# drprojects/DeepViewAgg

Hardware: AMD Instinct MI355X
Metric: points/sec fused fwd+bwd (1M pts, 32 views) (higher is better)
Workload: dtype bf16

## Files before the change

### deepviewagg_amd/_lib.py

```python
import ctypes
import os

_HERE = os.path.dirname(os.path.abspath(__file__))
LIB_PATH = os.environ.get("DVA_LIB_PATH") or os.path.join(_HERE, "csrc", "libdva_hip.so")

DVA_F32, DVA_BF16, DVA_F16 = 0, 1, 2
DVA_GRID_F32, DVA_GRID_F64, DVA_GRID_I32, DVA_GRID_I64 = 0, 1, 2, 3
DVA_SUM, DVA_MEAN, DVA_MAX, DVA_MIN = 0, 1, 2, 3
REDUCE_CODE = {"sum": DVA_SUM, "add": DVA_SUM, "mean": DVA_MEAN, "max": DVA_MAX, "min": DVA_MIN}
CAMERA_CODE = {
    "s3dis_equirectangular": 0,
    "scannet": 1,
    "kitti360_perspective": 2,
    "kitti360_fisheye": 3,
}

_ERRORS = {
    -1: "DVA_ERR_INVALID (bad argument)",
    -2: "DVA_ERR_UNSUPPORTED",
    -3: "DVA_ERR_LAUNCH (HIP runtime error)",
    -4: "DVA_ERR_OVERFLOW (composite key does not fit int64)",
}
DVA_ERR_UNSUPPORTED = -2

# ... 173 lines not shown
    "dva_copy_ceiling": (ctypes.c_int, [_vp, _vp, _i64, _vp]),
    "dva_zero_unseen_rows": (ctypes.c_int, [_vp, _vp, _i64, _i64, _vp]),
    "dva_chain_bn_consts": (ctypes.c_int, [_vp, ctypes.c_double, _vp, _vp, _vp, _vp, _vp, ctypes.c_float, ctypes.c_float,
                                           _i32, _vp, _i32, _i32, _vp, _vp, _vp]),
    "dva_concat_cast_fwd": (ctypes.c_int, [_vp, _vp, _vp, _i64, _i32, _i32, _i32, _vp]),
    "dva_concat_cast_bwd": (ctypes.c_int, [_vp, _vp, _vp, _i64, _i32, _i32, _i32, _vp]),
    "dva_mapping_row_index": (ctypes.c_int, [_vp, _vp, _vp, _i32, ctypes.c_double, _i64, _i64, _i32, _i32, _i32, _vp, _vp]),
    "dva_view_gather_rows_grad_rec16_to": (ctypes.c_int, [_vp, _vp, _vp, _vp, _vp, _i32, _i64, _i64, _i32, _i32, _i32, _vp]),
    "dva_chain_tile_chunks": (ctypes.c_int, [_vp, _i64, _i64, _i32, _vp, _vp]),
    "dva_chain_tile_offsets": (ctypes.c_int, [_vp, _i32, _vp, _vp, _vp]),
    "dva_bn_bwd_consts": (ctypes.c_int, [_vp, _vp, ctypes.c_double, _i32, _vp, _vp, _vp, _i32, _vp]),
    "dva_chain3_prep": (ctypes.c_int, [_vp, _vp, _vp, _i32, _vp, _vp, _i32, _vp, _vp]),
    "dva_chain3_stats2": (ctypes.c_int, [_vp] * 11 + [_i64, _vp]),
    "dva_chain3_stats": (ctypes.c_int, [_i32] + [_vp] * 9 + [_i64, _i64, _vp]),
    "dva_chain3_scores": (ctypes.c_int, [_vp] * 7 + [_i32, _vp, _i64, _vp]),
    "dva_chain3_score_stats": (ctypes.c_int, [_vp] * 10 + [_i32, _i64, _vp]),
    "dva_chain3_bwd_layer": (ctypes.c_int, [_i32] + [_vp] * 19 + [_i64, _i64, _vp]),
    "dva_chain_stats1": (ctypes.c_int, [_vp, _vp, _i32, _vp, _vp]),
    "dva_chain_dw1": (ctypes.c_int, [_vp, _vp, _vp, _i32, _vp, _vp, _vp, _vp]),
    "dva_chain_set_prep": (ctypes.c_int, [_vp, _i32, _vp, _vp, _i32, _vp, _vp]),
    "dva_chain_set_fwd": (ctypes.c_int, [_i32, _vp, _vp, _vp, _vp, _vp, _vp, _vp, _vp, _i64, _vp]),
    "dva_chain_set_bwd": (ctypes.c_int, [_i32, _vp, _vp, _vp, _vp, _vp, _vp, _vp, _vp, _vp, _vp, _vp, _i32, _vp, _vp,
                                         _i64, _vp]),
    "dva_chain3_set_prep": (ctypes.c_int, [_vp, _i32, _vp, _vp, _i32, _vp, _vp]),
    "dva_chain3_set_fwd": (ctypes.c_int, [_i32, _vp, _vp, _vp, _vp, _vp, _vp, _vp, _vp, _i64, _vp]),
    "dva_chain3_set_bwd": (ctypes.c_int, [_i32, _vp, _vp, _vp, _vp, _vp, _vp, _vp, _vp, _vp, _vp, _vp, _i32, _vp, _vp,
                                         _i64, _vp]),
    "dva_voxel_parent_workspace_bytes": (ctypes.c_int64, [_i64]),
    "dva_voxel_parent_index": (ctypes.c_int, [_vp, _i64, _vp, _i64, _i32, _i32, _vp, _vp, _i64, _vp]),
    "dva_voxel_kernel_map": (ctypes.c_int, [_vp, _i64, _vp, _i64, _vp, _i32, _vp, _vp, _i64, _vp]),
    "dva_sparse_conv_workspace_bytes": (ctypes.c_int64, [_i32, _i32, _i32, _i32]),
    "dva_sparse_conv_apply": (ctypes.c_int, [_vp, _vp, _vp, _vp, _vp, _i64, _i64, _i32, _i32, _i32, _i32, _i32, _vp,
                                             _i64, _vp]),
    "dva_sparse_conv_wgrad": (ctypes.c_int, [_vp, _vp, _vp, _vp, _i64, _i64, _i32, _i32, _i32, _i32, _vp]),
    "dva_knn_workspace_bytes": (ctypes.c_int64, [_i64]),
    "dva_knn": (ctypes.c_int, [_vp, _i64, _vp, _f32, _i32, _i32, _vp, _vp, _vp, _vp, _i64, _vp]),
    "dva_view_occlusion": (ctypes.c_int, [_vp, _vp, _i64, _i64, _i32, _vp, _i32, _vp, _i32, _vp, _vp, _vp]),
    "dva_knn_query_workspace_bytes": (ctypes.c_int64, [_i64, _i64]),
    "dva_knn_query": (ctypes.c_int, [_vp, _i64, _vp, _i64, _vp, _f32, _i32, _i32, _vp, _vp, _vp, _vp, _i64, _vp]),
    "dva_pointwise_pca": (ctypes.c_int, [_vp, _i64, _vp, _i64, _i32, _vp, _vp, _vp]),
    "dva_grid_workspace_bytes": (ctypes.c_int64, [_i64, _i64]),
    "dva_grid_quantize": (ctypes.c_int, [_vp, _i32, _i64, _f64, _vp, _vp, _vp, _vp, _i64, _vp]),
    "dva_grid_cluster": (ctypes.c_int, [_vp, _vp, _vp, _i64, _vp, _i32, _vp, _vp, _vp, _vp, _vp, _vp, _vp, _i64, _vp]),
    "dva_grid_mean": (ctypes.c_int, [_vp, _i32, _i64, _i32, _vp, _vp, _i64, _vp, _vp, _i64, _vp]),
    "dva_grid_majority": (ctypes.c_int, [_vp, _i64, _vp, _i64, _i64, _i64, _i32, _vp, _vp, _i64, _vp]),
    "dva_radius_query_workspace_bytes": (ctypes.c_int64, [_i64, _i64]),
# ... 178 lines not shown
```

### deepviewagg_amd/csrc/chain_set.hip

```cpp
#include "chain_split.h"

namespace dva {
namespace chain {

enum { SO_WSA = 0, SO_WSB = 4, SO_WCB = 8, SO_WCBT = 12, SO_WSBT = 16, SO_WSAT = 20, N_SOPS = 24 };

__global__ __launch_bounds__(64) void set_prep_kernel(const float* __restrict__ Wsa, int ldsa,
                                                      const float* __restrict__ Wsb, const float* __restrict__ Wc,
                                                      int ldc, uint4* __restrict__ ops) {
  const int op = blockIdx.x, lane = threadIdx.x, j = lane & 31, h = lane >> 5;
  const int mat = op / 4, lo = (op >> 1) & 1, m = op & 1;
  float w[8];
#pragma unroll
  for (int s = 0; s < 8; ++s) {
    const int c = chan(8 * m + s, h);
    float v;
    switch (mat) {
      case 0: v = Wsa[j * ldsa + c]; break;
      case 1: v = Wsb[j * D + c]; break;
      case 2: v = Wc[j * ldc + D + c]; break;
      case 3: v = Wc[c * ldc + D + j]; break;
      case 4: v = Wsb[c * D + j]; break;
      default: v = Wsa[c * ldsa + j]; break;
    }
    const float hi = bf2f(f2bf(v));
    w[s] = lo ? v - hi : hi;
  }
  ops[op * 64 + lane] = __builtin_bit_cast(uint4, pack8(w));
}

template <int DIR, int STAGE>
__global__ __launch_bounds__(256, DIR == 0 ? 4 : 3) void set_kernel(
    const float* __restrict__ pooled, const int64_t* __restrict__ ptr, const float* __restrict__ w33,
    const uint4* __restrict__ ops, const float* __restrict__ bn_s1, const float* __restrict__ bn_s2,
    const float* __restrict__ sm_s1, const float* __restrict__ sm_s2, const float* __restrict__ du,
    float* __restrict__ u_out, float* __restrict__ dpooled, float* __restrict__ dW, int ld_dw,
    float* __restrict__ dw33, double* __restrict__ stats, int64_t N) {
  __shared__ __attribute__((aligned(16))) float s_tab[2][TAB_FLOATS];
  __shared__ __attribute__((aligned(16))) float s_w33[D];
  __shared__ __attribute__((aligned(16))) uint4 s_ops[N_SOPS * 64];
  __shared__ __attribute__((aligned(16))) bf16_t s_ta[4][32 * TSB], s_tb[4][32 * TSB];
  __shared__ float s_red[D * D];
  const int lane = threadIdx.x & 63, wv = threadIdx.x >> 6, j = lane & 31, h = lane >> 5;
  for (int i = threadIdx.x; i < N_SOPS * 64; i += blockDim.x) s_ops[i] = ops[i];
  stage_tab(s_tab[0], bn_s1, (DIR == 1 && STAGE == 3) ? sm_s1 : nullptr, false);
  stage_tab(s_tab[1], bn_s2, (DIR == 1 && STAGE >= 2) ? sm_s2 : nullptr, false);
  for (int i = threadIdx.x; i < D; i += blockDim.x) s_w33[i] = w33 ? w33[chan(i & 15, i >> 4)] : 0.f;
  __syncthreads();
  const __amdgpu_buffer_rsrc_t PL = make_rsrc(pooled, (uint64_t)N * 128), DU = make_rsrc(du, (uint64_t)N * 128),
                               UO = make_rsrc(u_out, (uint64_t)N * 128), DPO = make_rsrc(dpooled, (uint64_t)N * 128);
  float st[2][16];
#pragma unroll
  for (int r = 0; r < 16; ++r) st[0][r] = st[1][r] = 0.f;
  f32x16 accW = {0};
  float acc33[16];
#pragma unroll
  for (int r = 0; r < 16; ++r) acc33[r] = 0.f;
  bf16_t* ta = s_ta[wv];
  bf16_t* tb = s_tb[wv];
  const f32x16 zero = {0};
  const int64_t tiles = (N + 31) / 32;
  const int64_t wave = rfl((int)(((int64_t)blockIdx.x * blockDim.x + threadIdx.x) >> 6));
  const int64_t n_waves = ((int64_t)gridDim.x * blockDim.x) >> 6;
  for (int64_t t = wave; t < tiles; t += n_waves) {
    const int64_t p = t * 32 + j;
    const bool ok = p < N;
    const uint32_t keep = ok ? 0xffffffffu : 0u, row = (uint32_t)p;
    float x[16], w3[16];
    load_rows16(PL, ok, row, h, x);
    float num = 0.f;
    if (w33 && ok) num = sqrtf(1.f / ((float)(ptr[p + 1] - ptr[p]) + 1e-3f));
    tab16(s_w33, 0, h, w3);
    const Split xs = split16(x, keep);
    f32x16 z1 = mm3(s_ops, SO_WSA, lane, xs, zero);
#pragma unroll
    for (int r = 0; r < 16; ++r) z1[r] = ok ? __builtin_fmaf(num, w3[r], z1[r]) : 0.f;
    auto add_stats = [&](const f32x16& z) {
#pragma unroll
      for (int r = 0; r < 16; ++r) {
        st[0][r] += z[r];
        st[1][r] = __builtin_fmaf(z[r], z[r], st[1][r]);
      }
    };
    if (DIR == 0 && STAGE == 1) { add_stats(z1); continue; }
    float a1[16], a2[16];
    act16(z1, s_tab[0], h, a1);
    const Split a1s = split16(a1, keep);
    const f32x16 z2 = mm3(s_ops, SO_WSB, lane, a1s, zero);
    if (DIR == 0 && STAGE == 2) { add_stats(z2); continue; }
    act16(z2, s_tab[1], h, a2);
    const Split a2s = split16(a2, keep);
    if (DIR == 0) {
      store_rows16(UO, ok, row, h, mm3(s_ops, SO_WCB, lane, a2s, zero));
      continue;
// ... 14 lines not shown
    layer_bwd<false, true>(z2, da2, s_tab[1], h, ok, unused_st, dz);
#pragma unroll
    for (int r = 0; r < 16; ++r) dz[r] = ok ? dz[r] : 0.f;
    const Split dz2s = split16(dz, keep);
    const f32x16 da1 = mm3(s_ops, SO_WSBT, lane, dz2s, zero);
    if (STAGE == 2) {
      float tmp[16];
      layer_bwd<true, false>(z1, da1, s_tab[0], h, ok, st, tmp);
      tileT_put_f32(ta, j, h, dz, ok);
      tileT_put_f32(tb, j, h, a1, ok);
      wave_sync();
      accW = wgrad(ta, tb, j, h, accW);
      wave_sync();
      continue;
    }
    float dz1[16];
    layer_bwd<false, true>(z1, da1, s_tab[0], h, ok, unused_st, dz1);
#pragma unroll
    for (int r = 0; r < 16; ++r) {
      dz1[r] = ok ? dz1[r] : 0.f;
      acc33[r] = __builtin_fmaf(dz1[r], num, acc33[r]);
    }
    const Split dz1s = split16(dz1, keep);
    store_rows16(DPO, ok, row, h, mm3(s_ops, SO_WSAT, lane, dz1s, zero));
    tileT_put_f32(ta, j, h, dz1, ok);
    tileT_put_f32(tb, j, h, x, ok);
    wave_sync();
    accW = wgrad(ta, tb, j, h, accW);
    wave_sync();
  }
  if (DIR == 1) flush_matrix(accW, dW, ld_dw, D, false, s_red);
  if (DIR == 1 && STAGE == 3 && dw33) {
    __syncthreads();
    for (int i = threadIdx.x; i < D; i += blockDim.x) s_red[i] = 0.f;
    __syncthreads();
#pragma unroll
    for (int r = 0; r < 16; ++r) {
      float v = acc33[r];
#pragma unroll
      for (int off = 1; off < 32; off <<= 1) v += __shfl_xor(v, off);
      if (j == 0) atomicAdd(&s_red[chan(r, h)], v);
    }
    __syncthreads();
    for (int i = threadIdx.x; i < D; i += blockDim.x) atomicAdd(&dw33[i * ld_dw], s_red[i]);
  }
  if (!(DIR == 0 && STAGE == 3) && !(DIR == 1 && STAGE == 3)) flush_stats<2>(st, stats, s_red);
}

}
}

using namespace dva;
using namespace dva::chain;

extern "C" {

int dva_chain_set_prep(const float* Wsa, int32_t ld_sa, const float* Wsb, const float* Wc, int32_t ld_c, void* ops,
                       void* stream) {
  if (!Wsa || !Wsb || !Wc || !ops || ld_sa < D || ld_c < 2 * D) return DVA_ERR_INVALID;
  hipLaunchKernelGGL(set_prep_kernel, dim3(N_SOPS), dim3(64), 0, (hipStream_t)stream, Wsa, ld_sa, Wsb, Wc, ld_c,
                     (uint4*)ops);
  DVA_CHECK_LAUNCH();
  return DVA_OK;
}

int dva_chain_set_fwd(int32_t stage, const float* pooled, const int64_t* ptr, const float* w33, const void* ops,
                      const float* bn_s1, const float* bn_s2, float* u, double* stats, int64_t n_points,
                      void* stream) {
  if (n_points < 0 || stage < 1 || stage > 3) return DVA_ERR_INVALID;
  if (n_points == 0) return DVA_OK;
  if (!pooled || !ptr || !ops || (stage >= 2 && !bn_s1) || (stage == 3 && (!bn_s2 || !u)) || (stage < 3 && !stats))
    return DVA_ERR_INVALID;
  if (n_points * 128 > 0xfffffff0ll) return DVA_ERR_UNSUPPORTED;
  const int64_t tiles = (n_points + 31) / 32;
  const int cap = chain_grid(2);
  const int64_t want = (tiles + 31) / 32;
  const dim3 grid((int)(want < cap ? want : cap)), block(256);
  hipStream_t s = (hipStream_t)stream;
  const float *b1 = bn_s1, *b2 = bn_s2;
#define DVA_SET_FWD(ST_)                                                                                          \
  hipLaunchKernelGGL((set_kernel<0, ST_>), grid, block, 0, s, pooled, ptr, w33, (const uint4*)ops, b1, b2,      \
                     (const float*)nullptr, (const float*)nullptr, (const float*)nullptr, u, (float*)nullptr,   \
                     (float*)nullptr, 0, (float*)nullptr, stats, n_points)
  if (stage == 1) DVA_SET_FWD(1);
  else if (stage == 2) DVA_SET_FWD(2);
  else DVA_SET_FWD(3);
#undef DVA_SET_FWD
  DVA_CHECK_LAUNCH();
  return DVA_OK;
}

int dva_chain_set_bwd(int32_t stage, const float* pooled, const int64_t* ptr, const float* w33, const void* ops,
                      const float* bn_s1, const float* bn_s2, const float* sm_s1, const float* sm_s2,
                      const float* du, float* dpooled, float* dW, int32_t ld_dw, float* dw33, double* stats,
                      int64_t n_points, void* stream) {
  if (n_points < 0 || stage < 1 || stage > 3) return DVA_ERR_INVALID;
  if (n_points == 0) return DVA_OK;
  if (!pooled || !ptr || !ops || !bn_s1 || !bn_s2 || !du || !dW || ld_dw < D || (stage < 3 && !stats) ||
      (stage >= 2 && !sm_s2) || (stage == 3 && (!sm_s1 || !dpooled)))
    return DVA_ERR_INVALID;
  if (n_points * 128 > 0xfffffff0ll) return DVA_ERR_UNSUPPORTED;
  const int64_t tiles = (n_points + 31) / 32;
  const int cap = chain_grid(2);
  const int64_t want = (tiles + 31) / 32;
  const dim3 grid((int)(want < cap ? want : cap)), block(256);
  hipStream_t s = (hipStream_t)stream;
#define DVA_SET_BWD(ST_)                                                                                          \
  hipLaunchKernelGGL((set_kernel<1, ST_>), grid, block, 0, s, pooled, ptr, w33, (const uint4*)ops, bn_s1, bn_s2, \
                     sm_s1, sm_s2, du, (float*)nullptr, dpooled, dW, ld_dw, dw33, stats, n_points)
  if (stage == 1) DVA_SET_BWD(1);
  else if (stage == 2) DVA_SET_BWD(2);
  else DVA_SET_BWD(3);
#undef DVA_SET_BWD
  DVA_CHECK_LAUNCH();
  return DVA_OK;
}

}
```

### deepviewagg_amd/csrc/segment.hip

```cpp
#include "dva_common.h"

namespace dva {

template <typename T, int REDUCE>
__global__ __launch_bounds__(256) void segment_csr_fwd_kernel(const T* __restrict__ src,
                                                               const int64_t* __restrict__ ptr,
                                                               T* __restrict__ out,
                                                               int32_t* __restrict__ arg,
                                                               int64_t n_groups, int C) {
  const int64_t total = n_groups * (int64_t)C;
  for (int64_t t = blockIdx.x * (int64_t)blockDim.x + threadIdx.x; t < total;
       t += (int64_t)gridDim.x * blockDim.x) {
    const int64_t g = t / C;
    const int c = (int)(t - g * C);
    const int64_t beg = ptr[g], end = ptr[g + 1];
    float acc;
    int64_t best = -1;
    if (REDUCE == DVA_SUM || REDUCE == DVA_MEAN) {
      acc = 0.f;
      for (int64_t r = beg; r < end; ++r) acc += Elt<T>::ld(src, r * C + c);
      if (REDUCE == DVA_MEAN && end > beg) acc /= (float)(end - beg);
    } else {
      acc = 0.f;
      for (int64_t r = beg; r < end; ++r) {
// ... 267 lines not shown
      hipLaunchKernelGGL((segment_csr_bwd_vec_kernel<T, R>), dim3(grid), dim3(256), 0, s, (const T*)gout, \
                         ptr, arg, (T*)gsrc, n, C);                                                      \
    else                                                                                                 \
      hipLaunchKernelGGL((segment_csr_bwd_kernel<T, R>), dim3(grid), dim3(256), 0, s, (const T*)gout,    \
                         ptr, arg, (T*)gsrc, n, C);                                                      \
  } while (0)
  switch (reduce) {
    case DVA_SUM: DVA_L(DVA_SUM); break;
    case DVA_MEAN: DVA_L(DVA_MEAN); break;
    case DVA_MAX: DVA_L(DVA_MAX); break;
    case DVA_MIN: DVA_L(DVA_MIN); break;
    default: return DVA_ERR_INVALID;
  }
#undef DVA_L
  return DVA_OK;
}

}

using namespace dva;

extern "C" {

int dva_version(void) { return 329; }

int dva_device_count(void) {
  int n = 0;
  hipError_t e = hipGetDeviceCount(&n);
  if (e == hipErrorNoDevice) return 0;
  if (e != hipSuccess) return DVA_ERR_LAUNCH;
  return n;
}

int dva_segment_csr_fwd(const void* src, const int64_t* ptr, void* out, int32_t* arg,
                        int64_t n_groups, int32_t C, int32_t dtype, int32_t reduce, void* stream) {
  if (n_groups < 0 || C < 0 || !ptr) return DVA_ERR_INVALID;
  if (reduce < DVA_SUM || reduce > DVA_MIN) return DVA_ERR_INVALID;
  if (n_groups == 0 || C == 0) return DVA_OK;
  if (!out) return DVA_ERR_INVALID;
  int rc;
  if (dtype == DVA_F32)
    rc = launch_segment_fwd<float>(src, ptr, out, arg, n_groups, C, reduce, (hipStream_t)stream);
  else if (dtype == DVA_BF16)
    rc = launch_segment_fwd<bf16_t>(src, ptr, out, arg, n_groups, C, reduce, (hipStream_t)stream);
  else if (dtype == DVA_F16)
    rc = launch_segment_fwd<f16_t>(src, ptr, out, arg, n_groups, C, reduce, (hipStream_t)stream);
  else
// ... 81 lines not shown
```

### deepviewagg_amd/fused_chain.py

```python
import collections
import os

import torch

from . import _lib, ops, fused_deepset
from ._lib import check, fits_buffer, ptr, require_device, stream_of
from .fused_deepset import D, _bn_of, _bn_consts

FORCE = None
VIEWS_PER_CHUNK = 512
OPS_BYTES = 18 * 64 * 16 + 7 * 64 * 32


def enabled():
    if FORCE is not None:
        return FORCE
    return torch.is_autocast_enabled('cuda') and torch.get_autocast_dtype('cuda') in (torch.bfloat16, torch.float16)


ROW_DTYPES = (torch.bfloat16, torch.float16)


def applicable(module, x_mod, x_map, csr_idx=None):
    if not enabled() or module.use_mod or module.save_last:
# ... 35 lines not shown
    check(lib.dva_chain_tile_count(ptr(csr_idx), ptr(cp), n_chunks, ptr(counts), st), "dva_chain_tile_count")
    check(lib.dva_chain_tile_offsets(ptr(counts), n_chunks, ptr(offsets), ptr(n_tiles), st),
          "dva_chain_tile_offsets")
    check(lib.dva_chain_tile_build(ptr(csr_idx), ptr(cp), n_chunks, ptr(offsets), ptr(tiles), st),
          "dva_chain_tile_build")
    return tiles, n_tiles


def _chain_bn(stats, m, bn, training, W=None, K=0, sum_a=None):
    lib = _lib.load()
    out = torch.empty((5, D), dtype=torch.float32, device=stats.device)
    fold = training and W is not None and sum_a is not None
    check(lib.dva_chain_bn_consts(ptr(stats), float(max(m, 1)), ptr(bn.running_mean), ptr(bn.running_var),
                                  ptr(bn.num_batches_tracked), ptr(bn.weight.detach()), ptr(bn.bias.detach()),
                                  float(bn.momentum), float(bn.eps), 1 if training else 0,
                                  ptr(W) if fold else None, W.shape[1] if fold else 0, K if fold else 0,
                                  ptr(sum_a) if fold else None, ptr(out), stream_of(stats)), "dva_chain_bn_consts")
    return out


SET_OPS_BYTES = 24 * 64 * 16


def _set_fns(lib, prec3):
    if prec3:
        return lib.dva_chain3_set_prep, lib.dva_chain3_set_fwd, lib.dva_chain3_set_bwd
    return lib.dva_chain_set_prep, lib.dva_chain_set_fwd, lib.dva_chain_set_bwd


def _set_branch_forward(e_map, pooled, csr_idx, training, zstats, prec3=False):
    lib = _lib.load()
    set_prep, set_fwd, _ = _set_fns(lib, prec3)
    dev, N = pooled.device, pooled.shape[0]
    st = stream_of(pooled)
    mlp_set = e_map.mlp_set
    Wc = e_map.mlp_elt_2[0][0].weight.detach().contiguous()
    Wsa = mlp_set[0][0].weight.detach().contiguous()
    Wsb = mlp_set[1][0].weight.detach().contiguous()
    set_bns = [_bn_of(mlp_set[0]), _bn_of(mlp_set[1])]
    w33 = Wsa[:, D].contiguous() if e_map.use_num else None
    sops = torch.empty(SET_OPS_BYTES, dtype=torch.uint8, device=dev)
    check(set_prep(ptr(Wsa), Wsa.shape[1], ptr(Wsb), ptr(Wc), Wc.shape[1], ptr(sops), st), "dva_chain_set_prep")
    su1, su2 = zstats(), zstats()
    if training:
        check(set_fwd(1, ptr(pooled), ptr(csr_idx), ptr(w33), ptr(sops), None, None, None, ptr(su1), N, st),
              "dva_chain_set_fwd")
    bns1 = _bn_consts(su1, N, set_bns[0], training)
    if training:
        check(set_fwd(2, ptr(pooled), ptr(csr_idx), ptr(w33), ptr(sops), ptr(bns1), None, None, ptr(su2), N, st),
              "dva_chain_set_fwd")
    bns2 = _bn_consts(su2, N, set_bns[1], training)
    t_add = torch.empty((N, D), dtype=torch.float32, device=dev)
    check(set_fwd(3, ptr(pooled), ptr(csr_idx), ptr(w33), ptr(sops), ptr(bns1), ptr(bns2), ptr(t_add), None, N, st),
          "dva_chain_set_fwd")
    return t_add, (pooled, csr_idx, w33, sops, bns1, bns2, tuple(Wsa.shape), prec3)


def _set_branch_backward(saved, dt, dWc, training, zstats, arena):
    from .fused_chain_bwd import bn_bwd_consts
    lib = _lib.load()
    pooled, csr_idx, w33, sops, bns1, bns2, wsa_shape, prec3 = saved
    set_bwd = _set_fns(lib, prec3)[2]
    dev, N = pooled.device, pooled.shape[0]
    st = stream_of(pooled)
    n_rows = float(max(N, 1))

    def call(stage, sm1, sm2, dpooled, dW, ld, dw33, stats):
        check(set_bwd(stage, ptr(pooled), ptr(csr_idx), ptr(w33), ptr(sops), ptr(bns1), ptr(bns2), ptr(sm1), ptr(sm2),
                      ptr(dt), ptr(dpooled), ptr(dW), ld, ptr(dw33), ptr(stats), N, st), "dva_chain_set_bwd")
    ss2, ss1 = zstats(), zstats()
    call(1, None, None, None, dWc[:, D:], dWc.shape[1], None, ss2)
    sms2, g2, b2 = bn_bwd_consts(lib, arena, ss2, bns2, n_rows, training, st)
    dWsb = arena.take(D, D)
    call(2, None, sms2, None, dWsb, D, None, ss1)
    sms1, g1, b1 = bn_bwd_consts(lib, arena, ss1, bns1, n_rows, training, st)
    dWsa = arena.take(*wsa_shape)
    dpooled = torch.empty((N, D), dtype=torch.float32, device=dev)
    call(3, sms1, sms2, dpooled, dWsa, wsa_shape[1], dWsa[:, D:] if w33 is not None else None, None)
    return dpooled, [dWsa, g1, b1, dWsb, g2, b2]


CHAIN_SAVED = ("vp", "tiles", "n_tiles", "wops", "t_add", "zstar", "arg", "mom", "bn1", "bn2", "bn5", "bn6")


class ChainState(collections.namedtuple(
        "ChainState", CHAIN_SAVED + ("W1", "G", "training", "bs", "gw", "gb", "set_saved"), defaults=(None,) * 4)):
    __slots__ = ()

    def saved(self):
        return self[:len(CHAIN_SAVED)]

    @classmethod
    def restore(cls, saved, W1, G, training):
        return cls(*saved, W1=W1, G=G, training=training)


def take_set_saved(ctx, say_released=False):
    set_saved, ctx.set_saved = ctx.set_saved, None
    if set_saved is None:
        why = ": its per-step workspaces are released after the first backward" if say_released else ""
        raise RuntimeError(f"the recompute chain's backward ran twice on the same graph{why} (retain_graph is not "
# ... 21 lines not shown

    zstats = iter(ops.zeros_small((11, 3 * D), torch.float64, dev)).__next__
    with ops._timed("chain_tiles", N * 8):
        tiles, n_tiles = build_tiles(csr_idx, V)
        vp = torch.empty(V, dtype=torch.int32, device=dev)
        check(lib.dva_csr_expand(ptr(csr_idx), N, ptr(vp), st), "dva_csr_expand")
    wops = torch.empty(OPS_BYTES, dtype=torch.uint8, device=dev)
    check(lib.dva_chain_prep(ptr(W1), ptr(W2), ptr(W5), W5.shape[1], ptr(W6), ptr(Ws), G, ptr(wops), st),
          "dva_chain_prep")
    s1 = zstats()
    mom = zstats()[:44]
    if training:
        with ops._timed("chain_moments", V * 32):
            check(lib.dva_chain_moments(ptr(x_map), V, ptr(W1), 0, ptr(mom), ptr(s1), st), "dva_chain_moments")
    bn1 = _chain_bn(s1, V, bns[0], training, W1, 8, mom)
    s2 = zstats()
    zstar = torch.empty((N, D), dtype=torch.float32, device=dev)
    arg = torch.empty((N, D), dtype=torch.int32, device=dev)
    with ops._timed("chain_stats2", V * 36 + N * 256):
        check(lib.dva_chain_stats2(ptr(x_map), ptr(vp), ptr(tiles), ptr(n_tiles), ptr(wops), ptr(bn1),
                                   ptr(bns[1].weight.detach()), ptr(s2), ptr(zstar), ptr(arg), V, st),
              "dva_chain_stats2")
    bn2 = _chain_bn(s2, V, bns[1], training, W2, D, s2[2 * D:])
    pooled = torch.empty((N, D), dtype=torch.float32, device=dev)
    check(lib.dva_chain_pooled(ptr(zstar), ptr(bn2), ptr(csr_idx), ptr(pooled), N, st), "dva_chain_pooled")
    t_add, set_saved = _set_branch_forward(e_map, pooled, csr_idx, training, zstats)
    s5, s6 = zstats(), zstats()
    if training:
        with ops._timed("chain_stats5", V * 36 + N * 128):
            check(lib.dva_chain_stats(5, ptr(x_map), ptr(vp), ptr(t_add), ptr(tiles), ptr(n_tiles), ptr(wops),
                                      ptr(bn1), ptr(bn2), None, ptr(s5), V, N, st), "dva_chain_stats")
    bn5 = _chain_bn(s5, V, bns[2], training)
    if training:
        with ops._timed("chain_stats6", V * 36 + N * 128):
            check(lib.dva_chain_stats(6, ptr(x_map), ptr(vp), ptr(t_add), ptr(tiles), ptr(n_tiles), ptr(wops),
                                      ptr(bn1), ptr(bn2), ptr(bn5), ptr(s6), V, N, st), "dva_chain_stats")
    bn6 = _chain_bn(s6, V, bns[3], training, W6, D, s6[2 * D:])
    return ChainState(vp=vp, tiles=tiles, n_tiles=n_tiles, wops=wops, t_add=t_add, zstar=zstar, arg=arg, mom=mom, bn1=bn1,
                      bn2=bn2, bn5=bn5, bn6=bn6, W1=W1, G=G, training=training, bs=bs, gw=gw, gb=gb, set_saved=set_saved)


class _ChainPool(torch.autograd.Function):

    @staticmethod
    def forward(ctx, rows, row_idx, plan, x_map, csr_idx, module, scaling, eps, *params):
        lib = _lib.load()
        require_device(rows, row_idx, x_map, csr_idx)
        rows = rows.contiguous()
        x_map = x_map.contiguous()
# ... 216 lines not shown
```

### deepviewagg_amd/fused_chain_bwd.py

```python
import torch

from . import _lib, ops
from ._lib import check, ptr, stream_of
from .fused_deepset import D


class Arena:

    def __init__(self, device, n_floats=1 << 15):
        self.buf = ops.zeros_small(n_floats, torch.float32, device)
        self.used = 0

    def take(self, *shape):
        n = 1
        for d in shape:
            n *= d
        off = self.used
        self.used = off + (n + 3) // 4 * 4
        assert self.used <= self.buf.numel(), "Arena too small"
        return self.buf[off:off + n].view(*shape)


def bn_bwd_consts(lib, arena, stats, bn, m_rows, training, st, hat=True, out=True, width=D):
    sm = dg = db = None
# ... 40 lines not shown
                                                    ptr(da_out), ptr(dW), ptr(stats), keys[1], keys[2], V, N, st),
                      "dva_chain_bwd_layer6_keys")
                return
            check(lib.dva_chain_bwd_layer(stage, ptr(x_map), ptr(vp), ptr(t_add), ptr(tiles), ptr(n_tiles), ptr(wops),
                                          ptr(bn1), ptr(bn2), ptr(bn5), ptr(bn6), ptr(sm2), ptr(sm5), ptr(sm6),
                                          ptr(dc), ptr(arg_), ptr(dpooled_), ptr(da_in), ptr(da_out), ptr(dW),
                                          ptr(du), ptr(P), ptr(stats), min(G, 4), V, N, st),
                  "dva_chain_bwd_layer")

    sm6, g6, b6 = consts(s6, bn6)
    dW6 = arena.take(D, D)
    s5 = zstats()
    da5 = torch.empty((V, D), dtype=torch.bfloat16, device=dev)
    layer(6, None, None, sm6, None, None, None, da5, dW6, None, None, s5, "chain_bwd_l6",
          V * (32 + 4 + 16 + 64) + N * 128)
    sm5, g5, b5 = consts(s5, bn5)
    dW5 = arena.take(D, 2 * D)
    du = torch.zeros((N, D), dtype=torch.float32, device=dev)
    s2 = zstats()
    da2 = torch.empty((V, D), dtype=torch.bfloat16, device=dev)
    layer(5, None, sm5, None, None, None, da5, da2, dW5, du, None, s2, "chain_bwd_l5",
          V * (32 + 4 + 64 + 64) + N * 256)
    del da5
    dpooled, d_set = _set_branch_backward(set_saved, du, dW5, training, zstats, arena)
    consts(s2, bn2, out=False)
    dpooled_dy = torch.empty((N, D), dtype=torch.float32, device=dev)
    check(lib.dva_chain_route_stats(ptr(S.zstar), ptr(dpooled), ptr(bn2), ptr(csr_idx), ptr(s2), ptr(dpooled_dy), N,
                                    st), "dva_chain_route_stats")
    sm2, g2, b2 = consts(s2, bn2, hat=False)
    dW2, P = arena.take(D, D), arena.take(D, 20)
    s1 = zstats()
    layer(2, sm2, None, None, S.arg, dpooled_dy, da2, None, dW2, None, P, None, "chain_bwd_l2",
          V * (32 + 4 + 64) + N * 256)
    del da2
    check(lib.dva_chain_stats1(ptr(P), ptr(S.W1), 0, ptr(s1), st), "dva_chain_stats1")
    sm1, g1, b1 = consts(s1, bn1)
    dW1 = arena.take(D, 8)
    check(lib.dva_chain_dw1(ptr(P), ptr(S.mom), ptr(S.W1), 0, ptr(bn1), ptr(sm1), ptr(dW1), st), "dva_chain_dw1")
    if gate is not None:
        gG = G if keys is None else keys[1]
        dgw, dgb = gwb[:gG].reshape(gate.weight.shape), gwb[gG:].reshape(gate.bias.shape)
    else:
        dgw = dgb = None
    return [dW1, g1, b1, dW2, g2, b2, dW5, g5, b5, dW6, g6, b6, dWs, dbs, dgw, dgb] + d_set


def backward(ctx, gout):
    from .fused_chain import ChainState, take_set_saved
    lib = _lib.load()
    set_saved = take_set_saved(ctx, say_released=True)
    qk = getattr(ctx, "qk", None)
# ... 41 lines not shown
```

### include/dva.h

```cpp
#ifndef DVA_H_
#define DVA_H_

#include <stdint.h>

#ifdef __cplusplus
extern "C" {
#endif

#define DVA_OK 0
#define DVA_ERR_INVALID (-1)
#define DVA_ERR_UNSUPPORTED (-2)
#define DVA_ERR_LAUNCH (-3)
#define DVA_ERR_OVERFLOW (-4)

#define DVA_F32 0
#define DVA_BF16 1
#define DVA_F16 2

#define DVA_SUM 0
#define DVA_MEAN 1
#define DVA_MAX 2
#define DVA_MIN 3

#define DVA_CAM_EQUIRECT 0
// ... 266 lines not shown
                      const float* gate_b, const void* grad_out, const void* out, float* grad_scores, void* view_rec,
                      float* grad_gate_wb, double* stats_b, const void* z_a, int64_t n_points, int64_t n_views,
                      int64_t n_rows, int32_t C_out, int32_t G, int32_t scaling, float eps, void* stream);
int dva_emod_bwd(int32_t stage, const void* Y, const int32_t* tap_rows, const float* tap_weights, const void* tiles,
                 const int32_t* n_tiles, const void* eops, const float* bn_a, const float* bn_b, const float* sm_a,
                 const float* sm_b, const void* view_rec, const void* grad_out, void* da, float* dWb, double* stats_a,
                 const void* z_a, int64_t n_points, int64_t n_views, int64_t n_rows, int32_t C_out, int32_t G,
                 void* stream);

int dva_bn_bwd_consts(double* stats, const float* bn, double inv_m, int32_t do_hat, float* sm, float* dgamma,
                      float* dbeta, int32_t C, void* stream);
int dva_chain_stats1(const float* P, const float* W1, int32_t exact_w1, double* stats, void* stream);
int dva_chain_dw1(const float* P, const double* mom, const float* W1, int32_t exact_w1, const float* bn1,
                  const float* sm1, float* dW1, void* stream);
int dva_chain_set_prep(const float* Wsa, int32_t ld_sa, const float* Wsb, const float* Wc, int32_t ld_c, void* ops,
                       void* stream);
int dva_chain_set_fwd(int32_t stage, const float* pooled, const int64_t* ptr, const float* w33, const void* ops,
                      const float* bn_s1, const float* bn_s2, float* u, double* stats, int64_t n_points,
                      void* stream);
int dva_chain_set_bwd(int32_t stage, const float* pooled, const int64_t* ptr, const float* w33, const void* ops,
                      const float* bn_s1, const float* bn_s2, const float* sm_s1, const float* sm_s2,
                      const float* du, float* dpooled, float* dW, int32_t ld_dw, float* dw33, double* stats,
                      int64_t n_points, void* stream);
int dva_chain_attn_bwd(const float* scores, const int32_t* view_point, const void* tiles, const int32_t* n_tiles,
                       const void* rows, const int32_t* row_idx, const int64_t* ptr, const float* gate_w,
                       const float* gate_b, const void* grad_out, const void* out, float* grad_scores, void* view_rec,
                       float* grad_gate_wb, int64_t n_points, int64_t n_views, int64_t n_rows, int32_t C, int32_t G,
                       int32_t scaling, float eps, void* stream);
int dva_chain_attn_bwd_dt(const float* scores, const int32_t* view_point, const void* tiles, const int32_t* n_tiles,
                          const void* rows, const int32_t* row_idx, const int64_t* ptr, const float* gate_w,
                          const float* gate_b, const void* grad_out, const void* out, float* grad_scores, void* view_rec,
                          float* grad_gate_wb, int64_t n_points, int64_t n_views, int64_t n_rows, int32_t C, int32_t G,
                          int32_t scaling, float eps, int32_t dtype, void* stream);
int dva_chain_attn_bwd_f32(const float* scores, const int32_t* view_point, const void* tiles, const int32_t* n_tiles,
                           const float* rows, const int32_t* row_idx, const int64_t* ptr, const float* gate_w,
                           const float* gate_b, const float* grad_out, const float* out, float* grad_scores,
                           float* view_rec, float* grad_gate_wb, int64_t n_points, int64_t n_views, int64_t n_rows,
                           int32_t C, int32_t G, int32_t scaling, float eps, void* stream);
int dva_chain_attn_fwd_keys(const float* x_map, const int32_t* view_point, const float* u, const void* tiles,
                            const int32_t* n_tiles, const void* ops, const float* bn1, const float* bn2,
                            const float* bn5, const float* bn6, const float* key_bias, const float* queries, float scale,
                            const void* rows, const int32_t* row_idx, const int64_t* ptr, const float* gate_w,
                            const float* gate_b, void* out, float* scores_out, void* keys_out, int64_t n_points,
                            int64_t n_views, int64_t n_rows, int32_t C, int32_t G, int32_t scaling, float eps,
                            void* stream);
int dva_chain_score_stats(const float* x_map, const int32_t* view_point, const float* u, const void* tiles,
// ... 322 lines not shown
```

Before: 107.1 million.

## Fuse pooled BN/leaky and route-stats into set-branch kernels

Drops the separate dva_chain_pooled kernel and the dva_chain_route_stats kernel. The set-branch kernels now read zstar directly, apply BN2 plus leaky ReLU on the fly, and in the stage-3 backward compute the routed gradient dy and the BN2 statistics inline. This removes two full N×D fp32 intermediate tensors and their passes over memory. In exchange, every set stage recomputes the pooled transform, a third BN table is staged in shared memory, and stage-3 backward occupancy is lowered to 2 blocks. The weight-gradient and dw33 reductions are also changed from atomics to a wave-ordered sum, which makes them deterministic but adds block barriers.

```diff
diff --git a/deepviewagg_amd/_lib.py b/deepviewagg_amd/_lib.py
--- a/deepviewagg_amd/_lib.py
+++ b/deepviewagg_amd/_lib.py
@@ -219,6 +219,8 @@
     "dva_chain_set_fwd": (ctypes.c_int, [_i32, _vp, _vp, _vp, _vp, _vp, _vp, _vp, _vp, _i64, _vp]),
     "dva_chain_set_bwd": (ctypes.c_int, [_i32, _vp, _vp, _vp, _vp, _vp, _vp, _vp, _vp, _vp, _vp, _vp, _i32, _vp, _vp,
                                          _i64, _vp]),
+    "dva_chain_set_fwd_z": (ctypes.c_int, [_i32] + [_vp] * 9 + [_i64, _vp]),
+    "dva_chain_set_bwd_z": (ctypes.c_int, [_i32] + [_vp] * 12 + [_i32, _vp, _vp, _i64, _vp]),
     "dva_chain3_set_prep": (ctypes.c_int, [_vp, _i32, _vp, _vp, _i32, _vp, _vp]),
     "dva_chain3_set_fwd": (ctypes.c_int, [_i32, _vp, _vp, _vp, _vp, _vp, _vp, _vp, _vp, _i64, _vp]),
     "dva_chain3_set_bwd": (ctypes.c_int, [_i32, _vp, _vp, _vp, _vp, _vp, _vp, _vp, _vp, _vp, _vp, _vp, _i32, _vp, _vp,
diff --git a/deepviewagg_amd/csrc/chain_set.hip b/deepviewagg_amd/csrc/chain_set.hip
--- a/deepviewagg_amd/csrc/chain_set.hip
+++ b/deepviewagg_amd/csrc/chain_set.hip
@@ -29,14 +29,61 @@
   ops[op * 64 + lane] = __builtin_bit_cast(uint4, pack8(w));
 }
 
-template <int DIR, int STAGE>
-__global__ __launch_bounds__(256, DIR == 0 ? 4 : 3) void set_kernel(
+__device__ __forceinline__ void pooled16(float (&x)[16], const float* tab, int h, bool seen) {
+  asm volatile("" ::: "memory");
+  float g[16], b[16];
+  tab16(tab, T_G, h, g);
+  tab16(tab, T_B, h, b);
+#pragma unroll
+  for (int r = 0; r < 16; ++r) x[r] = seen ? leaky(__builtin_fmaf(x[r], g[r], b[r])) : 0.f;
+}
+__device__ __forceinline__ void route16(const float (&z)[16], const f32x16& d, const float* tab, int h, bool seen,
+                                        float (&st)[2][16], float (&dy)[16]) {
+  asm volatile("" ::: "memory");
+#pragma unroll
+  for (int q = 0; q < 4; ++q) {
+    const int o = 16 * h + 4 * q;
+    const float4 g4 = *reinterpret_cast<const float4*>(tab + T_G * D + o);
+    const float4 b4 = *reinterpret_cast<const float4*>(tab + T_B * D + o);
+    const float4 i4 = *reinterpret_cast<const float4*>(tab + T_I * D + o);
+    const float4 m4 = *reinterpret_cast<const float4*>(tab + T_M * D + o);
+    const float g[4] = {g4.x, g4.y, g4.z, g4.w}, b[4] = {b4.x, b4.y, b4.z, b4.w};
+    const float iv[4] = {i4.x, i4.y, i4.z, i4.w}, mm[4] = {m4.x, m4.y, m4.z, m4.w};
+#pragma unroll
+    for (int e = 0; e < 4; ++e) {
+      const int r = 4 * q + e;
+      const float v = seen ? d[r] * dleaky(__builtin_fmaf(z[r], g[e], b[e])) : 0.f;
+      dy[r] = v;
+      st[0][r] += v;
+      st[1][r] = __builtin_fmaf(v, __builtin_fmaf(z[r], iv[e], mm[e]), st[1][r]);
+    }
+  }
+}
+
+__device__ __forceinline__ void flush_matrix_ordered(const f32x16& acc, float* __restrict__ out, int ld, float* s_red) {
+  const int lane = threadIdx.x & 63, wv = threadIdx.x >> 6, j = lane & 31, h = lane >> 5;
+  for (int w = 0; w < (int)(blockDim.x >> 6); ++w) {
+    __syncthreads();
+    if (wv == w) {
+#pragma unroll
+      for (int r = 0; r < 16; ++r) {
+        float* s = &s_red[chan(r, h) * D + j];
+        *s = w == 0 ? acc[r] : *s + acc[r];
+      }
+    }
+  }
+  __syncthreads();
+  flush_red(out, ld, D, false, s_red);
+}
+
+template <int DIR, int STAGE, bool FZ = false>
+__global__ __launch_bounds__(256, DIR == 0 ? 4 : (FZ && STAGE == 3) ? 2 : 3) void set_kernel(
     const float* __restrict__ pooled, const int64_t* __restrict__ ptr, const float* __restrict__ w33,
     const uint4* __restrict__ ops, const float* __restrict__ bn_s1, const float* __restrict__ bn_s2,
     const float* __restrict__ sm_s1, const float* __restrict__ sm_s2, const float* __restrict__ du,
     float* __restrict__ u_out, float* __restrict__ dpooled, float* __restrict__ dW, int ld_dw,
-    float* __restrict__ dw33, double* __restrict__ stats, int64_t N) {
-  __shared__ __attribute__((aligned(16))) float s_tab[2][TAB_FLOATS];
+    float* __restrict__ dw33, double* __restrict__ stats, int64_t N, const float* __restrict__ bn2) {
+  __shared__ __attribute__((aligned(16))) float s_tab[FZ ? 3 : 2][TAB_FLOATS];
   __shared__ __attribute__((aligned(16))) float s_w33[D];
   __shared__ __attribute__((aligned(16))) uint4 s_ops[N_SOPS * 64];
   __shared__ __attribute__((aligned(16))) bf16_t s_ta[4][32 * TSB], s_tb[4][32 * TSB];
@@ -45,6 +92,7 @@
   for (int i = threadIdx.x; i < N_SOPS * 64; i += blockDim.x) s_ops[i] = ops[i];
   stage_tab(s_tab[0], bn_s1, (DIR == 1 && STAGE == 3) ? sm_s1 : nullptr, false);
   stage_tab(s_tab[1], bn_s2, (DIR == 1 && STAGE >= 2) ? sm_s2 : nullptr, false);
+  if (FZ) stage_tab(s_tab[FZ ? 2 : 0], bn2, nullptr, false);
   for (int i = threadIdx.x; i < D; i += blockDim.x) s_w33[i] = w33 ? w33[chan(i & 15, i >> 4)] : 0.f;
   __syncthreads();
   const __amdgpu_buffer_rsrc_t PL = make_rsrc(pooled, (uint64_t)N * 128), DU = make_rsrc(du, (uint64_t)N * 128),
@@ -66,10 +114,20 @@
     const int64_t p = t * 32 + j;
     const bool ok = p < N;
     const uint32_t keep = ok ? 0xffffffffu : 0u, row = (uint32_t)p;
-    float x[16], w3[16];
+    float x[16], w3[16], zs[16];
     load_rows16(PL, ok, row, h, x);
     float num = 0.f;
-    if (w33 && ok) num = sqrtf(1.f / ((float)(ptr[p + 1] - ptr[p]) + 1e-3f));
+    bool seen = false;
+    if constexpr (FZ) {
+      const int64_t cnt = ok ? ptr[p + 1] - ptr[p] : 0;
+      seen = cnt > 0;
+      if (w33 && ok) num = sqrtf(1.f / ((float)cnt + 1e-3f));
+#pragma unroll
+      for (int r = 0; r < 16; ++r) zs[r] = seen ? x[r] : 0.f;
+      pooled16(x, s_tab[FZ ? 2 : 0], h, seen);
+    } else if (w33 && ok) {
+      num = sqrtf(1.f / ((float)(ptr[p + 1] - ptr[p]) + 1e-3f));
+    }
     tab16(s_w33, 0, h, w3);
     const Split xs = split16(x, keep);
     f32x16 z1 = mm3(s_ops, SO_WSA, lane, xs, zero);
@@ -130,29 +188,37 @@
       acc33[r] = __builtin_fmaf(dz1[r], num, acc33[r]);
     }
     const Split dz1s = split16(dz1, keep);
-    store_rows16(DPO, ok, row, h, mm3(s_ops, SO_WSAT, lane, dz1s, zero));
+    if constexpr (FZ) {
+      float dy[16];
+      route16(zs, mm3(s_ops, SO_WSAT, lane, dz1s, zero), s_tab[FZ ? 2 : 0], h, seen, st, dy);
+      store_rows16(DPO, ok, row, h, dy);
+    } else {
+      store_rows16(DPO, ok, row, h, mm3(s_ops, SO_WSAT, lane, dz1s, zero));
+    }
     tileT_put_f32(ta, j, h, dz1, ok);
     tileT_put_f32(tb, j, h, x, ok);
     wave_sync();
     accW = wgrad(ta, tb, j, h, accW);
     wave_sync();
   }
-  if (DIR == 1) flush_matrix(accW, dW, ld_dw, D, false, s_red);
+  if (DIR == 1) flush_matrix_ordered(accW, dW, ld_dw, s_red);
   if (DIR == 1 && STAGE == 3 && dw33) {
-    __syncthreads();
-    for (int i = threadIdx.x; i < D; i += blockDim.x) s_red[i] = 0.f;
-    __syncthreads();
 #pragma unroll
     for (int r = 0; r < 16; ++r) {
-      float v = acc33[r];
-#pragma unroll
-      for (int off = 1; off < 32; off <<= 1) v += __shfl_xor(v, off);
-      if (j == 0) atomicAdd(&s_red[chan(r, h)], v);
+#pragma unroll
+      for (int off = 1; off < 32; off <<= 1) acc33[r] += __shfl_xor(acc33[r], off);
+    }
+    for (int w = 0; w < (int)(blockDim.x >> 6); ++w) {
+      __syncthreads();
+      if (wv == w && j == 0) {
+#pragma unroll
+        for (int r = 0; r < 16; ++r) s_red[chan(r, h)] = w == 0 ? acc33[r] : s_red[chan(r, h)] + acc33[r];
+      }
     }
     __syncthreads();
     for (int i = threadIdx.x; i < D; i += blockDim.x) atomicAdd(&dw33[i * ld_dw], s_red[i]);
   }
-  if (!(DIR == 0 && STAGE == 3) && !(DIR == 1 && STAGE == 3)) flush_stats<2>(st, stats, s_red);
+  if (!(DIR == 0 && STAGE == 3) && !(DIR == 1 && STAGE == 3 && !FZ)) flush_stats<2>(st, stats, s_red);
 }
 
 }
@@ -172,24 +238,31 @@
   return DVA_OK;
 }
 
-int dva_chain_set_fwd(int32_t stage, const float* pooled, const int64_t* ptr, const float* w33, const void* ops,
-                      const float* bn_s1, const float* bn_s2, float* u, double* stats, int64_t n_points,
-                      void* stream) {
-  if (n_points < 0 || stage < 1 || stage > 3) return DVA_ERR_INVALID;
-  if (n_points == 0) return DVA_OK;
-  if (!pooled || !ptr || !ops || (stage >= 2 && !bn_s1) || (stage == 3 && (!bn_s2 || !u)) || (stage < 3 && !stats))
-    return DVA_ERR_INVALID;
-  if (n_points * 128 > 0xfffffff0ll) return DVA_ERR_UNSUPPORTED;
+}
+
+static dim3 set_grid(int64_t n_points) {
   const int64_t tiles = (n_points + 31) / 32;
   const int cap = chain_grid(2);
   const int64_t want = (tiles + 31) / 32;
-  const dim3 grid((int)(want < cap ? want : cap)), block(256);
+  return dim3((int)(want < cap ? want : cap));
+}
+
+template <bool FZ>
+static int set_fwd(int32_t stage, const float* src, const float* bn2, const int64_t* ptr, const float* w33,
+                   const void* ops, const float* bn_s1, const float* bn_s2, float* u, double* stats, int64_t n_points,
+                   void* stream) {
+  if (n_points < 0 || stage < 1 || stage > 3) return DVA_ERR_INVALID;
+  if (n_points == 0) return DVA_OK;
+  if (!src || (FZ && !bn2) || !ptr || !ops || (stage >= 2 && !bn_s1) || (stage == 3 && (!bn_s2 || !u)) ||
+      (stage < 3 && !stats))
+    return DVA_ERR_INVALID;
+  if (n_points * 128 > 0xfffffff0ll) return DVA_ERR_UNSUPPORTED;
+  const dim3 grid = set_grid(n_points), block(256);
   hipStream_t s = (hipStream_t)stream;
-  const float *b1 = bn_s1, *b2 = bn_s2;
 #define DVA_SET_FWD(ST_)                                                                                          \
-  hipLaunchKernelGGL((set_kernel<0, ST_>), grid, block, 0, s, pooled, ptr, w33, (const uint4*)ops, b1, b2,      \
-                     (const float*)nullptr, (const float*)nullptr, (const float*)nullptr, u, (float*)nullptr,   \
-                     (float*)nullptr, 0, (float*)nullptr, stats, n_points)
+  hipLaunchKernelGGL((set_kernel<0, ST_, FZ>), grid, block, 0, s, src, ptr, w33, (const uint4*)ops, bn_s1, bn_s2, \
+                     (const float*)nullptr, (const float*)nullptr, (const float*)nullptr, u, (float*)nullptr,    \
+                     (float*)nullptr, 0, (float*)nullptr, stats, n_points, bn2)
   if (stage == 1) DVA_SET_FWD(1);
   else if (stage == 2) DVA_SET_FWD(2);
   else DVA_SET_FWD(3);
@@ -198,24 +271,22 @@
   return DVA_OK;
 }
 
-int dva_chain_set_bwd(int32_t stage, const float* pooled, const int64_t* ptr, const float* w33, const void* ops,
-                      const float* bn_s1, const float* bn_s2, const float* sm_s1, const float* sm_s2,
-                      const float* du, float* dpooled, float* dW, int32_t ld_dw, float* dw33, double* stats,
-                      int64_t n_points, void* stream) {
+template <bool FZ>
+static int set_bwd(int32_t stage, const float* src, const float* bn2, const int64_t* ptr, const float* w33,
+                   const void* ops, const float* bn_s1, const float* bn_s2, const float* sm_s1, const float* sm_s2,
+                   const float* du, float* dpooled, float* dW, int32_t ld_dw, float* dw33, double* stats,
+                   int64_t n_points, void* stream) {
   if (n_points < 0 || stage < 1 || stage > 3) return DVA_ERR_INVALID;
   if (n_points == 0) return DVA_OK;
-  if (!pooled || !ptr || !ops || !bn_s1 || !bn_s2 || !du || !dW || ld_dw < D || (stage < 3 && !stats) ||
-      (stage >= 2 && !sm_s2) || (stage == 3 && (!sm_s1 || !dpooled)))
+  if (!src || (FZ && !bn2) || !ptr || !ops || !bn_s1 || !bn_s2 || !du || !dW || ld_dw < D ||
+      ((stage < 3 || FZ) && !stats) || (stage >= 2 && !sm_s2) || (stage == 3 && (!sm_s1 || !dpooled)))
     return DVA_ERR_INVALID;
   if (n_points * 128 > 0xfffffff0ll) return DVA_ERR_UNSUPPORTED;
-  const int64_t tiles = (n_points + 31) / 32;
-  const int cap = chain_grid(2);
-  const int64_t want = (tiles + 31) / 32;
-  const dim3 grid((int)(want < cap ? want : cap)), block(256);
+  const dim3 grid = set_grid(n_points), block(256);
   hipStream_t s = (hipStream_t)stream;
 #define DVA_SET_BWD(ST_)                                                                                          \
-  hipLaunchKernelGGL((set_kernel<1, ST_>), grid, block, 0, s, pooled, ptr, w33, (const uint4*)ops, bn_s1, bn_s2, \
-                     sm_s1, sm_s2, du, (float*)nullptr, dpooled, dW, ld_dw, dw33, stats, n_points)
+  hipLaunchKernelGGL((set_kernel<1, ST_, FZ>), grid, block, 0, s, src, ptr, w33, (const uint4*)ops, bn_s1, bn_s2, \
+                     sm_s1, sm_s2, du, (float*)nullptr, dpooled, dW, ld_dw, dw33, stats, n_points, bn2)
   if (stage == 1) DVA_SET_BWD(1);
   else if (stage == 2) DVA_SET_BWD(2);
   else DVA_SET_BWD(3);
@@ -224,4 +295,34 @@
   return DVA_OK;
 }
 
-}
+extern "C" {
+
+int dva_chain_set_fwd(int32_t stage, const float* pooled, const int64_t* ptr, const float* w33, const void* ops,
+                      const float* bn_s1, const float* bn_s2, float* u, double* stats, int64_t n_points,
+                      void* stream) {
+  return set_fwd<false>(stage, pooled, nullptr, ptr, w33, ops, bn_s1, bn_s2, u, stats, n_points, stream);
+}
+
+int dva_chain_set_bwd(int32_t stage, const float* pooled, const int64_t* ptr, const float* w33, const void* ops,
+                      const float* bn_s1, const float* bn_s2, const float* sm_s1, const float* sm_s2,
+                      const float* du, float* dpooled, float* dW, int32_t ld_dw, float* dw33, double* stats,
+                      int64_t n_points, void* stream) {
+  return set_bwd<false>(stage, pooled, nullptr, ptr, w33, ops, bn_s1, bn_s2, sm_s1, sm_s2, du, dpooled, dW, ld_dw, dw33,
+                        stats, n_points, stream);
+}
+
+int dva_chain_set_fwd_z(int32_t stage, const float* zstar, const float* bn2, const int64_t* ptr, const float* w33,
+                        const void* ops, const float* bn_s1, const float* bn_s2, float* u, double* stats,
+                        int64_t n_points, void* stream) {
+  return set_fwd<true>(stage, zstar, bn2, ptr, w33, ops, bn_s1, bn_s2, u, stats, n_points, stream);
+}
+
+int dva_chain_set_bwd_z(int32_t stage, const float* zstar, const float* bn2, const int64_t* ptr, const float* w33,
+                        const void* ops, const float* bn_s1, const float* bn_s2, const float* sm_s1,
+                        const float* sm_s2, const float* du, float* dpooled_dy, float* dW, int32_t ld_dw, float* dw33,
+                        double* stats, int64_t n_points, void* stream) {
+  return set_bwd<true>(stage, zstar, bn2, ptr, w33, ops, bn_s1, bn_s2, sm_s1, sm_s2, du, dpooled_dy, dW, ld_dw, dw33,
+                       stats, n_points, stream);
+}
+
+}
diff --git a/deepviewagg_amd/csrc/segment.hip b/deepviewagg_amd/csrc/segment.hip
--- a/deepviewagg_amd/csrc/segment.hip
+++ b/deepviewagg_amd/csrc/segment.hip
@@ -313,7 +313,7 @@
 
 extern "C" {
 
-int dva_version(void) { return 329; }
+int dva_version(void) { return 330; }
 
 int dva_device_count(void) {
   int n = 0;
diff --git a/deepviewagg_amd/fused_chain.py b/deepviewagg_amd/fused_chain.py
--- a/deepviewagg_amd/fused_chain.py
+++ b/deepviewagg_amd/fused_chain.py
@@ -81,15 +81,21 @@
 SET_OPS_BYTES = 24 * 64 * 16
 
 
-def _set_fns(lib, prec3):
+def _set_fns(lib, prec3, from_z=False):
     if prec3:
         return lib.dva_chain3_set_prep, lib.dva_chain3_set_fwd, lib.dva_chain3_set_bwd
+    if from_z:
+        return lib.dva_chain_set_prep, lib.dva_chain_set_fwd_z, lib.dva_chain_set_bwd_z
     return lib.dva_chain_set_prep, lib.dva_chain_set_fwd, lib.dva_chain_set_bwd
 
 
-def _set_branch_forward(e_map, pooled, csr_idx, training, zstats, prec3=False):
-    lib = _lib.load()
-    set_prep, set_fwd, _ = _set_fns(lib, prec3)
+def _set_branch_forward(e_map, pooled, csr_idx, training, zstats, prec3=False, bn2=None):
+    lib = _lib.load()
+    from_z = bn2 is not None
+    assert not (prec3 and from_z)
+    set_prep, set_fwd, _ = _set_fns(lib, prec3, from_z)
+    src = (ptr(pooled), ptr(bn2)) if from_z else (ptr(pooled),)
+    name = "dva_chain_set_fwd_z" if from_z else "dva_chain_set_fwd"
     dev, N = pooled.device, pooled.shape[0]
     st = stream_of(pooled)
     mlp_set = e_map.mlp_set
@@ -102,31 +108,32 @@
     check(set_prep(ptr(Wsa), Wsa.shape[1], ptr(Wsb), ptr(Wc), Wc.shape[1], ptr(sops), st), "dva_chain_set_prep")
     su1, su2 = zstats(), zstats()
     if training:
-        check(set_fwd(1, ptr(pooled), ptr(csr_idx), ptr(w33), ptr(sops), None, None, None, ptr(su1), N, st),
-              "dva_chain_set_fwd")
+        check(set_fwd(1, *src, ptr(csr_idx), ptr(w33), ptr(sops), None, None, None, ptr(su1), N, st), name)
     bns1 = _bn_consts(su1, N, set_bns[0], training)
     if training:
-        check(set_fwd(2, ptr(pooled), ptr(csr_idx), ptr(w33), ptr(sops), ptr(bns1), None, None, ptr(su2), N, st),
-              "dva_chain_set_fwd")
+        check(set_fwd(2, *src, ptr(csr_idx), ptr(w33), ptr(sops), ptr(bns1), None, None, ptr(su2), N, st), name)
     bns2 = _bn_consts(su2, N, set_bns[1], training)
     t_add = torch.empty((N, D), dtype=torch.float32, device=dev)
-    check(set_fwd(3, ptr(pooled), ptr(csr_idx), ptr(w33), ptr(sops), ptr(bns1), ptr(bns2), ptr(t_add), None, N, st),
-          "dva_chain_set_fwd")
-    return t_add, (pooled, csr_idx, w33, sops, bns1, bns2, tuple(Wsa.shape), prec3)
-
-
-def _set_branch_backward(saved, dt, dWc, training, zstats, arena):
+    check(set_fwd(3, *src, ptr(csr_idx), ptr(w33), ptr(sops), ptr(bns1), ptr(bns2), ptr(t_add), None, N, st), name)
+    return t_add, (pooled, csr_idx, w33, sops, bns1, bns2, tuple(Wsa.shape), prec3, bn2)
+
+
+def _set_branch_backward(saved, dt, dWc, training, zstats, arena, s2=None):
     from .fused_chain_bwd import bn_bwd_consts
     lib = _lib.load()
-    pooled, csr_idx, w33, sops, bns1, bns2, wsa_shape, prec3 = saved
-    set_bwd = _set_fns(lib, prec3)[2]
+    pooled, csr_idx, w33, sops, bns1, bns2, wsa_shape, prec3, bn2 = saved
+    from_z = bn2 is not None
+    assert from_z == (s2 is not None)
+    set_bwd = _set_fns(lib, prec3, from_z)[2]
+    src = (ptr(pooled), ptr(bn2)) if from_z else (ptr(pooled),)
+    name = "dva_chain_set_bwd_z" if from_z else "dva_chain_set_bwd"
     dev, N = pooled.device, pooled.shape[0]
     st = stream_of(pooled)
     n_rows = float(max(N, 1))
 
     def call(stage, sm1, sm2, dpooled, dW, ld, dw33, stats):
-        check(set_bwd(stage, ptr(pooled), ptr(csr_idx), ptr(w33), ptr(sops), ptr(bns1), ptr(bns2), ptr(sm1), ptr(sm2),
-                      ptr(dt), ptr(dpooled), ptr(dW), ld, ptr(dw33), ptr(stats), N, st), "dva_chain_set_bwd")
+        check(set_bwd(stage, *src, ptr(csr_idx), ptr(w33), ptr(sops), ptr(bns1), ptr(bns2), ptr(sm1), ptr(sm2),
+                      ptr(dt), ptr(dpooled), ptr(dW), ld, ptr(dw33), ptr(stats), N, st), name)
     ss2, ss1 = zstats(), zstats()
     call(1, None, None, None, dWc[:, D:], dWc.shape[1], None, ss2)
     sms2, g2, b2 = bn_bwd_consts(lib, arena, ss2, bns2, n_rows, training, st)
@@ -135,7 +142,7 @@
     sms1, g1, b1 = bn_bwd_consts(lib, arena, ss1, bns1, n_rows, training, st)
     dWsa = arena.take(*wsa_shape)
     dpooled = torch.empty((N, D), dtype=torch.float32, device=dev)
-    call(3, sms1, sms2, dpooled, dWsa, wsa_shape[1], dWsa[:, D:] if w33 is not None else None, None)
+    call(3, sms1, sms2, dpooled, dWsa, wsa_shape[1], dWsa[:, D:] if w33 is not None else None, s2)
     return dpooled, [dWsa, g1, b1, dWsb, g2, b2]
 
 
@@ -203,9 +210,7 @@
                                    ptr(bns[1].weight.detach()), ptr(s2), ptr(zstar), ptr(arg), V, st),
               "dva_chain_stats2")
     bn2 = _chain_bn(s2, V, bns[1], training, W2, D, s2[2 * D:])
-    pooled = torch.empty((N, D), dtype=torch.float32, device=dev)
-    check(lib.dva_chain_pooled(ptr(zstar), ptr(bn2), ptr(csr_idx), ptr(pooled), N, st), "dva_chain_pooled")
-    t_add, set_saved = _set_branch_forward(e_map, pooled, csr_idx, training, zstats)
+    t_add, set_saved = _set_branch_forward(e_map, zstar, csr_idx, training, zstats, bn2=bn2)
     s5, s6 = zstats(), zstats()
     if training:
         with ops._timed("chain_stats5", V * 36 + N * 128):
diff --git a/deepviewagg_amd/fused_chain_bwd.py b/deepviewagg_amd/fused_chain_bwd.py
--- a/deepviewagg_amd/fused_chain_bwd.py
+++ b/deepviewagg_amd/fused_chain_bwd.py
@@ -86,11 +86,8 @@
     layer(5, None, sm5, None, None, None, da5, da2, dW5, du, None, s2, "chain_bwd_l5",
           V * (32 + 4 + 64 + 64) + N * 256)
     del da5
-    dpooled, d_set = _set_branch_backward(set_saved, du, dW5, training, zstats, arena)
     consts(s2, bn2, out=False)
-    dpooled_dy = torch.empty((N, D), dtype=torch.float32, device=dev)
-    check(lib.dva_chain_route_stats(ptr(S.zstar), ptr(dpooled), ptr(bn2), ptr(csr_idx), ptr(s2), ptr(dpooled_dy), N,
-                                    st), "dva_chain_route_stats")
+    dpooled_dy, d_set = _set_branch_backward(set_saved, du, dW5, training, zstats, arena, s2=s2)
     sm2, g2, b2 = consts(s2, bn2, hat=False)
     dW2, P = arena.take(D, D), arena.take(D, 20)
     s1 = zstats()
diff --git a/include/dva.h b/include/dva.h
--- a/include/dva.h
+++ b/include/dva.h
@@ -312,6 +312,13 @@
                       const float* bn_s1, const float* bn_s2, const float* sm_s1, const float* sm_s2,
                       const float* du, float* dpooled, float* dW, int32_t ld_dw, float* dw33, double* stats,
                       int64_t n_points, void* stream);
+int dva_chain_set_fwd_z(int32_t stage, const float* zstar, const float* bn2, const int64_t* ptr, const float* w33,
+                        const void* ops, const float* bn_s1, const float* bn_s2, float* u, double* stats,
+                        int64_t n_points, void* stream);
+int dva_chain_set_bwd_z(int32_t stage, const float* zstar, const float* bn2, const int64_t* ptr, const float* w33,
+                        const void* ops, const float* bn_s1, const float* bn_s2, const float* sm_s1,
+                        const float* sm_s2, const float* du, float* dpooled_dy, float* dW, int32_t ld_dw, float* dw33,
+                        double* stats, int64_t n_points, void* stream);
 int dva_chain_attn_bwd(const float* scores, const int32_t* view_point, const void* tiles, const int32_t* n_tiles,
                        const void* rows, const int32_t* row_idx, const int64_t* ptr, const float* gate_w,
                        const float* gate_b, const void* grad_out, const void* out, float* grad_scores, void* view_rec,
```

New measurement: 108.1 million, median of 6. No clear change (+1.0%).
